# NicholasMilef/UUO-Mocap

Hardware: AMD Instinct MI355X
Metric: mocap frames/sec fitted (300-frame seq, 50 markers) (higher is better)
Workload: dtype f32

## Files before the change

uuo_mocap_amd/_lib.py:

```python
from __future__ import annotations

import ctypes
import os
import re
from ctypes import POINTER, c_char_p, c_float, c_int, c_int32, c_void_p

_HERE = os.path.dirname(os.path.abspath(__file__))
LIB_PATH = os.path.join(_HERE, "libuuo_hip.so")
HEADER_PATH = os.path.join(os.path.dirname(_HERE), "include", "uuo_hip.h")

UUO_STAGE_CHAMFER, UUO_STAGE_MARKER, UUO_STAGE_PART = 0, 1, 2


ABI_VERSION = 3


class UuoProblem(ctypes.Structure):
    _fields_ = [
        ("stage", c_int32), ("F", c_int32), ("M", c_int32),
        ("d_markers", c_void_p), ("d_o_pose", c_void_p), ("d_o_betas", c_void_p), ("d_root", c_void_p),
        ("d_assign", c_void_p), ("d_subset", c_void_p), ("n_subset", c_int32),
        ("w_data", c_float), ("w_pose", c_float), ("w_betas", c_float), ("marker_distance", c_float),
        ("pose_cache_id", ctypes.c_uint64),
        ("w_soft", c_float), ("soft_tau", c_float),
        ("n_corners", c_int32), ("d_bary", c_void_p),
        ("robust_sigma", c_float),
    ]
    w_offsets = None


class _TailFloat:

    size = 4

    def __init__(self, offset: int):
        self.offset = offset

    def __get__(self, obj, owner=None):
        if obj is None:
            return self
        return c_float.from_buffer(obj, self.offset).value

    def __set__(self, obj, value):
        c_float.from_buffer(obj, self.offset).value = value


UuoProblem.w_offsets = _TailFloat(UuoProblem.robust_sigma.offset + 4)
assert UuoProblem.w_offsets.offset + 4 <= ctypes.sizeof(UuoProblem)


class UuoLbfgsOptions(ctypes.Structure):
    _fields_ = [
        ("max_iter", c_int32), ("history_size", c_int32), ("lr", c_float), ("tolerance_grad", c_float),
        ("tolerance_change", c_float), ("max_eval", c_int32), ("verbose", c_int32),
    ]


class UuoLbfgsStats(ctypes.Structure):
    _fields_ = [
        ("n_iter", c_int32), ("n_eval", c_int32), ("first_loss", c_float), ("final_loss", c_float),
        ("stop_reason", c_int32), ("device_ms", c_float),
    ]


class UuoReprojectionProblem(ctypes.Structure):
    _fields_ = [
        ("F", c_int32), ("M", c_int32), ("V", c_int32), ("J", c_int32),
        ("d_markers", c_void_p), ("d_joints0", c_void_p), ("d_verts0", c_void_p), ("d_kp_target", c_void_p),
        ("d_mask", c_void_p), ("focal", c_float * 2), ("center", c_float * 2),
        ("w_reprojection", c_float), ("w_chamfer", c_float),
    ]


EVAL_CALLBACK = ctypes.CFUNCTYPE(None, c_void_p, c_int, c_float, c_void_p)
GATHER_FN = ctypes.CFUNCTYPE(c_int, c_void_p, POINTER(ctypes.c_double), c_int, POINTER(ctypes.c_double))


class UuoShared(ctypes.Structure):
    _fields_ = [("gather", GATHER_FN), ("user", c_void_p), ("rank", c_int32), ("world", c_int32)]


_SIGNATURES = {
    "uuo_last_error": (c_char_p, []),
    "uuo_abi_version": (c_int, []),
    "uuo_model_create": (c_int, [c_void_p] * 7 + [c_int, POINTER(c_void_p)]),
    "uuo_model_destroy": (c_int, [c_void_p]),
    "uuo_model_num_verts": (c_int, [c_void_p]),
    "uuo_model_set_faces": (c_int, [c_void_p, c_void_p, c_int]),
    "uuo_ring_table": (c_int, [c_void_p, c_int, c_int, c_void_p, c_void_p]),
    "uuo_ring_closest_points": (c_int, [c_void_p, c_void_p, c_int, c_int, c_void_p, c_void_p, c_void_p, c_void_p, c_void_p,
                                        c_void_p, c_void_p]),
    "uuo_fit_set_surface": (c_int, [c_void_p, c_int32, c_float]),
    "uuo_fit_surface_corners": (c_int, [c_void_p, c_void_p, c_void_p, c_void_p]),
    "uuo_smpl_forward": (c_int, [c_void_p, c_void_p, c_int, c_void_p, c_void_p, c_int, c_void_p, c_void_p,
                                 c_void_p, c_void_p]),
    "uuo_smpl_backward": (c_int, [c_void_p, c_void_p, c_int, c_void_p, c_void_p, c_int, c_void_p, c_void_p, c_void_p,
                                  c_void_p, c_void_p, c_void_p, c_void_p, c_void_p, c_void_p]),
    "uuo_nn_argmin": (c_int, [c_void_p, c_int, c_int, c_int, c_void_p, c_void_p, c_void_p, c_int, c_void_p,
                              c_void_p, c_void_p]),
    "uuo_rigid_distance_std": (c_int, [c_void_p, c_int, c_int, c_void_p, c_void_p]),
    "uuo_assign_mean_argmin": (c_int, [c_void_p, c_int, c_int, c_int, c_void_p, c_void_p, c_void_p, c_void_p,
                                       c_void_p]),
    "uuo_soft_nn_forward": (c_int, [c_void_p, c_int, c_int, c_int, c_void_p, c_void_p, c_float, c_void_p, c_void_p,
                                    c_void_p, c_void_p]),
    "uuo_soft_nn_backward": (c_int, [c_void_p, c_int, c_int, c_int, c_void_p, c_void_p, c_float, c_void_p, c_void_p,
                                     c_void_p, c_void_p, c_void_p]),
    "uuo_copy_to_host": (c_int, [c_void_p, c_void_p, c_void_p, c_int]),
    "uuo_mesh_closest_points": (c_int, [c_void_p, c_int, c_int, c_int, c_int, c_void_p, c_void_p, c_void_p, c_void_p,
                                        c_void_p, c_void_p, c_void_p]),
    "uuo_fit_create": (c_int, [c_void_p, c_int, c_int, POINTER(c_void_p)]),
    "uuo_fit_destroy": (c_int, [c_void_p]),
    "uuo_assign_segments_argmin": (c_int, [c_void_p, c_int, c_int, c_int, c_int, c_void_p, c_void_p, c_void_p, c_void_p,
                                           c_void_p, c_void_p]),
    "uuo_fit_set_frame_assign": (c_int, [c_void_p, c_void_p]),
    "uuo_fit_set_joint_accel": (c_int, [c_void_p, c_float]),
    "uuo_fit_set_foot_lock": (c_int, [c_void_p, c_float, c_void_p]),
    "uuo_fit_set_floor": (c_int, [c_void_p, c_float, c_float, c_float, c_void_p, c_int, c_int, c_void_p]),
    "uuo_fit_set_capsules": (c_int, [c_void_p, c_float, c_int, c_void_p, c_void_p, c_int, c_void_p]),
    "uuo_fit_set_joint_limits": (c_int, [c_void_p, c_float, c_void_p, c_void_p]),
    "uuo_fit_set_prior_weights": (c_int, [c_void_p, c_void_p]),
    "uuo_problem_num_params": (c_int, [POINTER(UuoProblem)]),
    "uuo_closure_eval": (c_int, [c_void_p, c_void_p, POINTER(UuoProblem), c_void_p, c_void_p, c_void_p, c_void_p]),
    "uuo_lbfgs_solve": (c_int, [c_void_p, c_void_p, POINTER(UuoProblem), c_void_p, POINTER(UuoLbfgsOptions),
                                POINTER(UuoLbfgsStats), c_void_p, c_void_p]),
    "uuo_lbfgs_solve_shared": (c_int, [c_void_p, c_void_p, POINTER(UuoProblem), c_void_p, POINTER(UuoLbfgsOptions),
                                       POINTER(UuoLbfgsStats), POINTER(UuoShared), c_void_p, c_void_p]),
    "uuo_time_closure": (c_int, [c_void_p, c_void_p, POINTER(UuoProblem), c_void_p, c_int, c_int,
                                 POINTER(c_float)]),
    "uuo_lbfgs_minimize": (c_int, [c_void_p, c_int, c_void_p, POINTER(UuoLbfgsOptions), POINTER(UuoLbfgsStats), c_void_p,
                                   c_void_p, c_void_p, c_void_p]),
    "uuo_reprojection_create": (c_int, [POINTER(UuoReprojectionProblem), POINTER(c_void_p)]),
    "uuo_reprojection_destroy": (c_int, [c_void_p]),
    "uuo_reprojection_num_params": (c_int, [POINTER(UuoReprojectionProblem)]),
    "uuo_reprojection_eval": (c_int, [c_void_p, c_void_p, c_void_p, c_void_p, c_void_p, c_void_p, c_void_p]),
    "uuo_reprojection_solve": (c_int, [c_void_p, c_void_p, c_void_p, POINTER(UuoLbfgsOptions), POINTER(UuoLbfgsStats),
                                       c_void_p, c_void_p, c_void_p, c_void_p]),
    "uuo_set_wait_policy": (c_int, [c_int, c_int]),
    "uuo_mailbox_open": (c_int, [c_char_p, c_int32, c_int32, ctypes.c_double, POINTER(c_void_p)]),
    "uuo_mailbox_close": (c_int, [c_void_p]),
    "uuo_mailbox_gather": (c_int, [c_void_p, c_void_p, c_int, c_void_p]),
    "uuo_mailbox_stats": (c_int, [c_void_p, POINTER(ctypes.c_ulonglong), POINTER(ctypes.c_ulonglong)]),
    "uuo_copy_device": (c_int, [c_void_p, c_void_p, c_void_p, ctypes.c_size_t]),
    "uuo_batch_create": (c_int, [c_void_p, c_int, c_int, c_int, c_int, POINTER(c_void_p)]),
    "uuo_batch_destroy": (c_int, [c_void_p]),
    "uuo_batch_solve": (c_int, [c_void_p, c_void_p, POINTER(UuoProblem), POINTER(c_void_p), c_int,
                                POINTER(UuoLbfgsOptions), POINTER(UuoLbfgsStats)]),
    "uuo_batch_part_scores": (c_int, [c_void_p, c_void_p, POINTER(UuoProblem), POINTER(c_void_p), c_int,
                                      POINTER(c_float)]),
}
LIB_DEBUG_PATH = os.path.join(_HERE, "libuuo_hip_debug.so")
_DEBUG_SIGNATURES = {
    "uuo_lbfgs_selftest": (c_int, [c_void_p, c_int, c_int, c_void_p, POINTER(UuoLbfgsOptions),
                                   POINTER(UuoLbfgsStats), c_void_p, c_void_p]),
    "uuo_debug_fit_buffers": (c_int, [c_void_p, c_void_p, c_void_p]),
    "uuo_debug_nn_flags": (c_int, [c_void_p, c_void_p]),
    "uuo_debug_skin16_check": (c_int, [c_void_p, c_int]),
    "uuo_debug_small_coeffs": (c_int, [c_int, c_int, c_int, c_void_p]),
    "uuo_debug_time_small": (c_int, [c_int, c_int, c_int, POINTER(c_float)]),
    "uuo_debug_index_map": (c_int, [c_int, c_int, c_int, c_void_p]),
    "uuo_debug_problem_index_map": (c_int, [POINTER(UuoProblem), c_int, c_void_p]),
    "uuo_debug_bwd_select": (c_int, [c_void_p, c_int, c_void_p, c_void_p]),
    "uuo_debug_last_solve_n": (c_int, [c_void_p]),
    "uuo_debug_staging_script": (c_int, [c_void_p, c_int, ctypes.c_longlong, c_void_p]),
    "uuo_debug_lb_replay_create": (c_int, [c_int, c_int, POINTER(c_void_p)]),
    "uuo_debug_lb_replay_step": (c_int, [c_void_p, c_void_p, c_float, c_float, c_void_p, c_void_p, c_void_p, c_void_p]),
    "uuo_debug_lb_replay_state": (c_int, [c_void_p, c_void_p, c_void_p, c_void_p, c_int, c_void_p, c_void_p]),
    "uuo_debug_lb_replay_destroy": (c_int, [c_void_p]),
}

CLOSURE_FN = ctypes.CFUNCTYPE(c_int, c_void_p, c_void_p, c_void_p, c_void_p, c_void_p)

_lib = None
_lib_debug = None


def header_symbols():
    text = open(HEADER_PATH).read()
    text = re.sub(r"/\*.*?\*/", "", text, flags=re.S)
    names = re.findall(r"\b(uuo_[a-z0-9_]+)\s*\(", text)
    return sorted(set(n for n in names if n != "uuo_eval_callback_t"))


def load():
    global _lib
    if _lib is not None:
        return _lib
    if not os.path.isfile(LIB_PATH):
        raise RuntimeError(
            "libuuo_hip.so is missing (%s): run `python __graft_entry__.py` to build the HIP extension. "
            "There is no CPU fallback for the fitted path." % LIB_PATH)
    lib = ctypes.CDLL(LIB_PATH)
    for name in header_symbols():
        if not hasattr(lib, name):
            raise RuntimeError("libuuo_hip.so does not export %s declared in include/uuo_hip.h" % name)
    for name, (res, args) in _SIGNATURES.items():
        fn = getattr(lib, name)
        fn.restype = res
        fn.argtypes = args
    if lib.uuo_abi_version() != ABI_VERSION:
        raise RuntimeError("libuuo_hip.so has ABI version %d, this package binds version %d: rebuild it "
                           "(python __graft_entry__.py)" % (lib.uuo_abi_version(), ABI_VERSION))
    _lib = lib
    return lib


def load_debug():
    global _lib_debug
    if _lib_debug is not None:
        return _lib_debug
    if not os.path.isfile(LIB_DEBUG_PATH):
        raise RuntimeError("libuuo_hip_debug.so is missing (%s): run `python __graft_entry__.py`" % LIB_DEBUG_PATH)
    lib = ctypes.CDLL(LIB_DEBUG_PATH)
    for name, (res, args) in list(_SIGNATURES.items()) + list(_DEBUG_SIGNATURES.items()):
        fn = getattr(lib, name)
        fn.restype = res
        fn.argtypes = args
    _lib_debug = lib
    return lib


def check(rc: int, what: str = ""):
    if rc != 0:
        msg = load().uuo_last_error()
        raise RuntimeError("%s failed (%d): %s" % (what or "libuuo_hip call", rc, msg.decode() if msg else ""))
```

uuo_mocap_amd/csrc/nn_kernels.hip:

```cpp
#include <cstdlib>

#include "frame_math.h"

#define UUO_INF __builtin_huge_valf()
#include "tri_math.h"

__device__ __forceinline__ float uuo_sqrt_rn(float x) { return __builtin_sqrtf(x); }
__device__ __forceinline__ float uuo_div_rn(float x, float y) { return x / y; }

__device__ __forceinline__ unsigned long long pack_key(float d, unsigned idx) {
  return ((unsigned long long)__float_as_uint(d) << 32) | (unsigned long long)idx;
}

__device__ __forceinline__ float sqdist(float qx, float qy, float qz, float px, float py, float pz) {
  const float dx = __fsub_rn(qx, px), dy = __fsub_rn(qy, py), dz = __fsub_rn(qz, pz);
  return __fadd_rn(__fadd_rn(__fmul_rn(dx, dx), __fmul_rn(dy, dy)), __fmul_rn(dz, dz));
}

__device__ __forceinline__ void nn_body(const float* __restrict__ x, const float* __restrict__ y,
                                        const int* __restrict__ ysub, int P1, int P2, int nc, int S,
                                        unsigned long long* __restrict__ out, int n, int qg, int s) {
  __shared__ float4 sc[64];
  const int lane = threadIdx.x;
  const int q = qg * 64 + lane;
// ... 447 lines not shown
      pf2 T2[6];
      float4 ww;
      unsigned pj;
      float o[3];
      pso_skin(Cf, SB4, sA, sTr, v, cl, o, T2, ww, pj);
      const float rx = o[0] - sTr[0], ry = o[1] - sTr[1];
      if (!valid) o[0] = o[1] = o[2] = 1.0e18f;
      const unsigned cidv = valid ? (unsigned)c : 0xFFFFFFFFu;
      const pf2 ox2 = pf2{o[0], o[0]}, oy2 = pf2{o[1], o[1]}, oz2 = pf2{o[2], o[2]};
      float ax = 0.f, ay = 0.f, az = 0.f;
#pragma unroll
      for (int k = 0; k < QP; ++k) {
        const pf2 dx = qx[k] - ox2, dy = qy[k] - oy2, dz = qz[k] - oz2;
        const pf2 d2 = ((dx * dx) + (dy * dy)) + (dz * dz);
#pragma unroll
        for (int h = 0; h < 2; ++h) {
          const int q = 2 * k + h;
          if (q < QB) {
            const float d = h ? d2.y : d2.x;
            float p = PSO_EXP((uM[q] - d) * kexp) * uW[q];
            p += (cidv == uI[q]) ? c_hard : 0.f;
            ax = fmaf(p, h ? dx.y : dx.x, ax);
            ay = fmaf(p, h ? dy.y : dy.x, ay);
            az = fmaf(p, h ? dz.y : dz.x, az);
          }
        }
      }
      const float g0 = -ax, g1 = -ay, g2 = -az;
      if (!__any((ax != 0.f) | (ay != 0.f) | (az != 0.f))) continue;
      gs[0] += g0;
      gs[1] += g1;
      gs[2] += g2;
      tq += rx * g1 - ry * g0;
      const float dv0 = fmaf(T2[4].x, g2, fmaf(T2[2].x, g1, T2[0].x * g0));
      const float dv1 = fmaf(T2[4].y, g2, fmaf(T2[2].y, g1, T2[0].y * g0));
      const float dv2 = fmaf(T2[5].x, g2, fmaf(T2[3].x, g1, T2[1].x * g0));
      const float* svf = reinterpret_cast<const float*>(sv);
#pragma unroll
      for (int k = 0; k < 10; ++k) db[k] += fmaf(svf[20 + k], dv2, fmaf(svf[10 + k], dv1, svf[k] * dv0));
      const float wv[4] = {ww.x, ww.y, ww.z, ww.w};
#pragma unroll
      for (int n = 0; n < 4; ++n) {
        float* col = sF + ((pj >> (8 * n)) & 0xFFu) * 64u + tid;
        col[0] += wv[n] * g0;
        col[64] += wv[n] * g1;
        col[128] += wv[n] * g2;
      }
    }
  }
  float* pre = a.pre + (size_t)f * UUO_PRE;
  const float r1 = wave_sum_fast(gs[0]), r2 = wave_sum_fast(gs[1]), r3 = wave_sum_fast(gs[2]), r14 = wave_sum_fast(tq);
  float rb[10];
#pragma unroll
  for (int k = 0; k < 10; ++k) rb[k] = wave_sum_fast(db[k]);
  if (tid == 0) {
    pre[0] = loss;
    pre[1] = r1;
    pre[2] = r2;
    pre[3] = r3;
#pragma unroll
    for (int k = 0; k < 10; ++k) pre[4 + k] = rb[k];
    pre[14] = r14;
    pre[15] = 0.f;
  }
  __syncthreads();
  for (int t = tid; t < UUO_NUM_JOINTS * 3; t += 64) {
    float acc = 0.f;
#pragma unroll 8
    for (int i = 0; i < 64; ++i) acc += sF[t * 64 + ((i + t) & 63)];
    pre[16 + t] = acc;
  }
}
template <int QB>
__global__ __launch_bounds__(64) void k_part_soft(PartSoftArgs a) {
  const int f = (int)(blockIdx.x >> 3) * 8 + (int)(blockIdx.x & 7);
  if (f >= a.F) return;
  part_soft_body<QB>(a, f);
}
template <int QB>
__global__ __launch_bounds__(64) void k_part_soft_b(const PartSoftArgs* __restrict__ batch, int count) {
  const int r = (int)(blockIdx.x >> 3);
  const PartSoftArgs a = batch[r % count];
  const int f = (r / count) * 8 + (int)(blockIdx.x & 7);
  if (f >= a.F) return;
  part_soft_body<QB>(a, f);
}

int uuo_launch_part_soft(const uuo_model* m, hipStream_t s, int F, int P1, const float* cache, const float* sb, const float* A,
                         const float* trans, const int32_t* subset, int n_subset, const float* markers,
                         unsigned long long* packed, float* pre, float w_hard, float w_soft, float tau) {
  UUO_REQUIRE(P1 >= 1 && P1 <= NNQ_MAX && subset && n_subset > 0 && F > 0 && pre, "uuo_launch_part_soft: bad arguments");
  UUO_REQUIRE(tau > 0.f && w_soft != 0.f, "uuo_launch_part_soft: needs a positive temperature and a soft weight");
  const double fm = (double)F * (double)P1;
  PartSoftArgs a{{F, P1}, F, m->V, n_subset, P1, subset, cache, sb, A, trans, markers, m->ST, packed, pre,
                 (float)(1.4426950408889634 / (double)tau), (float)((double)tau * 0.6931471805599453), w_hard, w_soft,
                 (float)(2.0 * (double)w_hard / fm), (float)(2.0 * (double)w_soft / fm)};
  if (uuo_record(UUO_OP_PART_SOFT, F, P1, a)) return 0;
  const dim3 grid(8 * ((F + 7) / 8));
  switch (P1) {
#define PSO_CASE(Q) case Q: hipLaunchKernelGGL(k_part_soft<Q>, grid, dim3(64), 0, s, a); break;
    PSO_CASE(1) PSO_CASE(2) PSO_CASE(3) PSO_CASE(4) PSO_CASE(5) PSO_CASE(6) PSO_CASE(7) PSO_CASE(8)
    PSO_CASE(9) PSO_CASE(10) PSO_CASE(11) PSO_CASE(12) PSO_CASE(13) PSO_CASE(14) PSO_CASE(15) PSO_CASE(16)
#undef PSO_CASE
  }
  UUO_HIP_CHECK(hipGetLastError());
  return 0;
}

static int fill_keys(hipStream_t s, unsigned long long* packed, size_t count) {
  FillArgs f{{(int)((count + 255) / 256), 1}, packed, (int)count};
  if (uuo_record(UUO_OP_FILL, f.h.gx, 1, f)) return 0;
  UUO_HIP_CHECK(hipMemsetAsync(packed, 0xFF, count * sizeof(unsigned long long), s));
  return 0;
}

int uuo_launch_nn(hipStream_t s, int N, int P1, int P2, const float* x, const float* y, const int32_t* ysub, int P2s,
                  unsigned long long* packed) {
  const int nc = ysub ? P2s : P2;
  if (nc > 0 && N > 0 && P1 > 0 && P1 <= NNQ_MAX) {
    int S = 1;
    if (N < 1024) S = (1024 + N - 1) / N;
    const int maxS = (nc + 1023) / 1024;
    if (S > maxS) S = maxS;
    if (S < 1 || uuo_recorder) S = 1;
    if (S > 1) {
      const int rc = fill_keys(s, packed, (size_t)N * P1);
      if (rc) return rc;
    }
    NnArgs a{{N, S}, x, y, ysub, P1, P2, nc, S, packed};
    if (uuo_record(UUO_OP_NN_FEWQ, N, S, a)) return 0;
    hipLaunchKernelGGL(k_nn_fewq, dim3(N, S), dim3(256), 0, s, a);
    UUO_HIP_CHECK(hipGetLastError());
    return 0;
  }
  {
    const int rc = fill_keys(s, packed, (size_t)N * P1);
    if (rc) return rc;
  }
  if (nc <= 0 || N <= 0 || P1 <= 0) return 0;
  const int qgroups = (P1 + 63) / 64;
  int S = 1;
  const long waves = (long)N * qgroups;
  if (waves < 4096) S = (int)((4096 + waves - 1) / waves);
  const int maxS = (nc + 255) / 256;
  if (S > maxS) S = maxS;
  if (S < 1) S = 1;
  NnArgs a{{N, qgroups * S}, x, y, ysub, P1, P2, nc, S, packed};
  if (uuo_record(UUO_OP_NN, N, qgroups * S, a)) return 0;
  hipLaunchKernelGGL(k_nn, dim3(N, qgroups, S), dim3(64), 0, s, a);
  UUO_HIP_CHECK(hipGetLastError());
  return 0;
}

#define CULL_CAP 3072
#define CULL_CAP2 1024
#define CULL_MG 64
#define CULL_MAXU 512
#define CULL_UB 4
#define CULL_MAXG 8
#ifndef CULL_SUPER
#define CULL_SUPER 8
#endif
#ifndef CULL_T
#define CULL_T 256
#endif
__device__ __forceinline__ void nn_cull_body(int M, int V, int nunits, int mper, const float* __restrict__ x,
                                             const float* __restrict__ verts, const float* __restrict__ bbox,
                                             unsigned long long* __restrict__ packed, int* __restrict__ stats) {
  __builtin_amdgcn_s_setprio(1);
  __shared__ float sbox[CULL_MAXU * 6];
  __shared__ float smx[CULL_MG * 3];
  __shared__ float sub[CULL_MG];
  __shared__ unsigned long long skey[CULL_MG];
  __shared__ unsigned slist[CULL_CAP];
  __shared__ unsigned scount, scount2;
  const int f = blockIdx.x, tid = threadIdx.x, wave = tid >> 6, lane = tid & 63;
  const int m0 = blockIdx.y * mper;
  const int mg = min(mper, M - m0);
  if (mg <= 0) return;
  const float* vf = verts + (size_t)f * V * 3;
  {
    const float* bf = bbox + (size_t)f * nunits * 6;
    for (int i = tid; i < nunits * 6; i += CULL_T) sbox[i] = bf[i];
  }
  if (tid < mg) {
    const float* px = x + ((size_t)f * M + m0 + tid) * 3;
    const float qx = px[0], qy = px[1], qz = px[2];
    smx[tid * 3] = qx;
    smx[tid * 3 + 1] = qy;
    smx[tid * 3 + 2] = qz;
    unsigned prev = (unsigned)(packed[(size_t)f * M + m0 + tid] & 0xFFFFFFFFull);
    if (prev >= (unsigned)V) prev = 0;
    const float* pv = vf + (size_t)prev * 3;
    const unsigned long long key = pack_key(sqdist(qx, qy, qz, pv[0], pv[1], pv[2]), prev);
    skey[tid] = key;
    sub[tid] = __uint_as_float((unsigned)(key >> 32));
  }
  if (tid == 0) scount = 0u;
  if (tid == 1) scount2 = 0u;
  __syncthreads();
#if CULL_SUPER
  constexpr int NSUP_MAX = (CULL_MAXU + CULL_SUPER - 1) / CULL_SUPER;
  __shared__ float ssup[NSUP_MAX * 6];
  __shared__ unsigned slist2[CULL_CAP2];
  const int nsup = (nunits + CULL_SUPER - 1) / CULL_SUPER;
  for (int sidx = tid; sidx < nsup * 6; sidx += CULL_T) {
    const int sp = sidx / 6, c = sidx - sp * 6;
    const int u0 = sp * CULL_SUPER, u1 = min(nunits, u0 + CULL_SUPER);
    float v = sbox[u0 * 6 + c];
    for (int u = u0 + 1; u < u1; ++u) v = (c < 3) ? fminf(v, sbox[u * 6 + c]) : fmaxf(v, sbox[u * 6 + c]);
    ssup[sidx] = v;
  }
  __syncthreads();
  for (int e = tid; e < nsup * mg; e += CULL_T) {
    const int sp = e / mg, m = e - sp * mg;
    const float* b = ssup + sp * 6;
    const float qx = smx[m * 3], qy = smx[m * 3 + 1], qz = smx[m * 3 + 2];
    const float dx = fmaxf(fmaxf(__fsub_rn(b[0], qx), __fsub_rn(qx, b[3])), 0.f);
    const float dy = fmaxf(fmaxf(__fsub_rn(b[1], qy), __fsub_rn(qy, b[4])), 0.f);
    const float dz = fmaxf(fmaxf(__fsub_rn(b[2], qz), __fsub_rn(qz, b[5])), 0.f);
    const float lb = __fadd_rn(__fadd_rn(__fmul_rn(dx, dx), __fmul_rn(dy, dy)), __fmul_rn(dz, dz));
    if (lb <= sub[m]) {
      const unsigned pos = atomicAdd(&scount2, 1u);
      if (pos < CULL_CAP2) slist2[pos] = ((unsigned)m << 16) | (unsigned)sp;
    }
  }
  __syncthreads();
  const int found2 = (int)scount2;
  if (found2 > CULL_CAP2 && tid == 0) scount = CULL_CAP + 1u;
  for (int e = tid; e < min(found2, CULL_CAP2 + 0) * CULL_SUPER && found2 <= CULL_CAP2; e += CULL_T) {
    const unsigned ent = slist2[e / CULL_SUPER];
    const int m = (int)(ent >> 16), u = (int)(ent & 0xFFFFu) * CULL_SUPER + (e % CULL_SUPER);
    if (u < nunits) {
      const float* b = sbox + u * 6;
      const float qx = smx[m * 3], qy = smx[m * 3 + 1], qz = smx[m * 3 + 2];
      const float dx = fmaxf(fmaxf(__fsub_rn(b[0], qx), __fsub_rn(qx, b[3])), 0.f);
      const float dy = fmaxf(fmaxf(__fsub_rn(b[1], qy), __fsub_rn(qy, b[4])), 0.f);
      const float dz = fmaxf(fmaxf(__fsub_rn(b[2], qz), __fsub_rn(qz, b[5])), 0.f);
      const float lb = __fadd_rn(__fadd_rn(__fmul_rn(dx, dx), __fmul_rn(dy, dy)), __fmul_rn(dz, dz));
      if (lb <= sub[m]) {
        const unsigned pos = atomicAdd(&scount, 1u);
        if (pos < CULL_CAP) slist[pos] = ((unsigned)m << 16) | (unsigned)u;
      }
    }
  }
#else
  for (int u = tid; u < nunits; u += CULL_T) {
    const float* b = sbox + u * 6;
    const float b0 = b[0], b1 = b[1], b2 = b[2], b3 = b[3], b4 = b[4], b5 = b[5];
    unsigned long long mask = 0ull;
#pragma unroll 4
    for (int m = 0; m < mg; ++m) {
      const float qx = smx[m * 3], qy = smx[m * 3 + 1], qz = smx[m * 3 + 2];
      const float dx = fmaxf(fmaxf(__fsub_rn(b0, qx), __fsub_rn(qx, b3)), 0.f);
      const float dy = fmaxf(fmaxf(__fsub_rn(b1, qy), __fsub_rn(qy, b4)), 0.f);
      const float dz = fmaxf(fmaxf(__fsub_rn(b2, qz), __fsub_rn(qz, b5)), 0.f);
      const float lb = __fadd_rn(__fadd_rn(__fmul_rn(dx, dx), __fmul_rn(dy, dy)), __fmul_rn(dz, dz));
      mask |= (lb <= sub[m]) ? (1ull << m) : 0ull;
    }
    const int cnt = __popcll(mask);
    if (cnt) {
      unsigned pos = atomicAdd(&scount, (unsigned)cnt);
      while (mask) {
        const int m = __ffsll((long long)mask) - 1;
        mask &= mask - 1;
        if (pos < CULL_CAP) slist[pos] = ((unsigned)m << 16) | (unsigned)u;
        ++pos;
      }
    }
  }
#endif
  __syncthreads();
  const int found = (int)scount;
  const bool overflow = found > CULL_CAP;
  const int nent = overflow ? nunits * mg : found;
  for (int e0 = wave * 4 * CULL_UB; e0 < nent; e0 += (CULL_T / 64) * 4 * CULL_UB) {
    unsigned long long key[CULL_UB];
    int mm[CULL_UB];
    float vx[CULL_UB], vy[CULL_UB], vz[CULL_UB];
    int vid[CULL_UB];
#pragma unroll
    for (int r = 0; r < CULL_UB; ++r) {
      const int e = e0 + 4 * r + (lane >> 4);
      mm[r] = 0;
      vid[r] = -1;
      vx[r] = vy[r] = vz[r] = 0.f;
      if (e < nent) {
        int u;
        if (overflow) {
          u = e / mg;
          mm[r] = e - u * mg;
        } else {
          const unsigned ent = slist[e];
          mm[r] = (int)(ent >> 16);
          u = (int)(ent & 0xFFFFu);
        }
        const int vtx = u * 16 + (lane & 15);
        if (vtx < V) {
          const float* pv = vf + (size_t)vtx * 3;
          vx[r] = pv[0];
          vy[r] = pv[1];
          vz[r] = pv[2];
          vid[r] = vtx;
        }
      }
    }
#pragma unroll
    for (int r = 0; r < CULL_UB; ++r) {
      const int m = mm[r];
      key[r] = (vid[r] >= 0)
                   ? pack_key(sqdist(smx[m * 3], smx[m * 3 + 1], smx[m * 3 + 2], vx[r], vy[r], vz[r]), (unsigned)vid[r])
                   : ~0ull;
#pragma unroll
      for (int off = 8; off >= 1; off >>= 1) {
        const unsigned long long o = __shfl_xor(key[r], off, 16);
        key[r] = o < key[r] ? o : key[r];
      }
      if ((lane & 15) == 0 && key[r] != ~0ull) atomicMin(&skey[m], key[r]);
    }
  }
  __syncthreads();
  if (tid < mg) packed[(size_t)f * M + m0 + tid] = skey[tid];
  if (tid == 0 && stats) stats[f * CULL_MAXG + blockIdx.y] = overflow ? -found : found;
}

struct NnCullArgs {
  UuoGridHdr h;
  int M, V, nunits, mper;
  uuo_gptr<const float> x;
  uuo_gptr<const float> verts;
  uuo_gptr<const float> bbox;
  uuo_gptr<unsigned long long> packed;
  uuo_gptr<int> stats;
};
__global__ __launch_bounds__(CULL_T) void k_nn_cull(NnCullArgs a) {
  nn_cull_body(a.M, a.V, a.nunits, a.mper, a.x, a.verts, a.bbox, a.packed, a.stats);
}
__global__ __launch_bounds__(CULL_T) void k_nn_cull_b(const NnCullArgs* __restrict__ batch) {
  UUO_BATCH_PICK(NnCullArgs, batch)
  nn_cull_body(a.M, a.V, a.nunits, a.mper, a.x, a.verts, a.bbox, a.packed, a.stats);
}

int uuo_launch_nn_cull(hipStream_t s, int F, int M, int V, int nunits, const float* markers, const float* verts,
                       const float* bbox, unsigned long long* packed, int* stats) {
  if (F <= 0 || M <= 0) return 0;
  UUO_REQUIRE(nunits <= CULL_MAXU, "uuo_launch_nn_cull: too many vertex units for the LDS box table");
  int G = (M + CULL_MG - 1) / CULL_MG;
  while (G < CULL_MAXG && (long)F * G < 1024 && (M + G) / (G + 1) >= 8) ++G;
  const int mper = (M + G - 1) / G;
  UUO_REQUIRE(mper <= CULL_MG && G <= CULL_MAXG, "uuo_launch_nn_cull: too many markers per frame for the pruned search");
  NnCullArgs a{{F, G}, M, V, nunits, mper, markers, verts, bbox, packed, stats};
  if (uuo_record(UUO_OP_NN_CULL, F, G, a)) return 0;
  hipLaunchKernelGGL(k_nn_cull, dim3(F, G), dim3(CULL_T), 0, s, a);
  UUO_HIP_CHECK(hipGetLastError());
  return 0;
}

int uuo_batched_launch_nn(int op, hipStream_t s, const void* d_args, int count, int gx, int gy) {
  if (op == UUO_OP_FILL) {
    hipLaunchKernelGGL(k_fill_keys_b, dim3(gx, gy, count), dim3(256), 0, s, (const FillArgs*)d_args);
  } else if (op == UUO_OP_NN) {
    hipLaunchKernelGGL(k_nn_b, dim3(gx, gy, count), dim3(64), 0, s, (const NnArgs*)d_args);
  } else if (op == UUO_OP_NN_FEWQ) {
    hipLaunchKernelGGL(k_nn_fewq_b, dim3(gx, gy, count), dim3(256), 0, s, (const NnArgs*)d_args);
  } else if (op == UUO_OP_NN_CULL) {
    hipLaunchKernelGGL(k_nn_cull_b, dim3(gx, gy, count), dim3(CULL_T), 0, s, (const NnCullArgs*)d_args);
  } else if (op == UUO_OP_PART_FWD) {
    const dim3 grid(8 * ((gx + 7) / 8) * count);
    const PartFwdArgs* pa = (const PartFwdArgs*)d_args;
    switch (gy) {
#define PFW_CASE(Q) case Q: hipLaunchKernelGGL(k_part_fwd_b<Q>, grid, dim3(PFW_T), 0, s, pa, count); break;
      PFW_CASE(1) PFW_CASE(2) PFW_CASE(3) PFW_CASE(4) PFW_CASE(5) PFW_CASE(6) PFW_CASE(7) PFW_CASE(8)
      PFW_CASE(9) PFW_CASE(10) PFW_CASE(11) PFW_CASE(12) PFW_CASE(13) PFW_CASE(14) PFW_CASE(15) PFW_CASE(16)
#undef PFW_CASE
      default: UUO_REQUIRE(false, "batched k_part_fwd: markers per frame out of range");
    }
  } else if (op == UUO_OP_PART_SOFT) {
    const dim3 grid(8 * ((gx + 7) / 8) * count);
    const PartSoftArgs* pa = (const PartSoftArgs*)d_args;
    switch (gy) {
#define PSO_CASE(Q) case Q: hipLaunchKernelGGL(k_part_soft_b<Q>, grid, dim3(64), 0, s, pa, count); break;
      PSO_CASE(1) PSO_CASE(2) PSO_CASE(3) PSO_CASE(4) PSO_CASE(5) PSO_CASE(6) PSO_CASE(7) PSO_CASE(8)
      PSO_CASE(9) PSO_CASE(10) PSO_CASE(11) PSO_CASE(12) PSO_CASE(13) PSO_CASE(14) PSO_CASE(15) PSO_CASE(16)
#undef PSO_CASE
      default: UUO_REQUIRE(false, "batched k_part_soft: markers per frame out of range");
    }
  } else {
    return 1;
  }
  UUO_HIP_CHECK(hipGetLastError());
  return 0;
}

__global__ void k_nn_unpack(int count, const unsigned long long* __restrict__ packed, float* __restrict__ dist,
                            int32_t* __restrict__ idx) {
  const int i = blockIdx.x * blockDim.x + threadIdx.x;
  if (i >= count) return;
  const unsigned long long k = packed[i];
  if (dist) dist[i] = __uint_as_float((unsigned)(k >> 32));
  if (idx) idx[i] = (int32_t)(unsigned)(k & 0xFFFFFFFFull);
}

int uuo_launch_nn_unpack(hipStream_t s, int count, const unsigned long long* packed, float* dist, int32_t* idx) {
  if (count <= 0) return 0;
  hipLaunchKernelGGL(k_nn_unpack, dim3((count + 255) / 256), dim3(256), 0, s, count, packed, dist, idx);
  UUO_HIP_CHECK(hipGetLastError());
  return 0;
}

extern "C" int uuo_nn_argmin(void* stream, int N, int P1, int P2, const float* d_x, const float* d_y,
                             const int32_t* d_y_subset, int P2s, float* d_dist, int32_t* d_idx, void* d_ws) {
  UUO_REQUIRE(d_x && d_y && d_ws, "uuo_nn_argmin: null argument (workspace of N*P1 uint64 is required)");
  UUO_REQUIRE(N >= 0 && P1 >= 0 && P2 >= 0, "uuo_nn_argmin: negative size");
  hipStream_t s = (hipStream_t)stream;
  int rc = uuo_launch_nn(s, N, P1, P2, d_x, d_y, d_y_subset, P2s, (unsigned long long*)d_ws);
  if (rc) return rc;
  return uuo_launch_nn_unpack(s, N * P1, (const unsigned long long*)d_ws, d_dist, d_idx);
}

#define ASSIGN_MG 4
#define ASSIGN_FC 32
#define ASSIGN_U 4
__global__ __launch_bounds__(256) void k_assign(int F, int M, int V, const float* __restrict__ verts,
                                                 const float* __restrict__ markers,
                                                 const unsigned char* __restrict__ valid, int count,
                                                 unsigned long long* __restrict__ out) {
  __shared__ float sm[ASSIGN_FC][ASSIGN_MG * 3];
  __shared__ unsigned char sv[ASSIGN_FC];
  const int v = blockIdx.x * 256 + threadIdx.x;
  const int vc = v < V ? v : V - 1;
  const int m0 = blockIdx.y * ASSIGN_MG;
  float acc[ASSIGN_MG];
#pragma unroll
  for (int g = 0; g < ASSIGN_MG; ++g) acc[g] = 0.f;
  for (int f0 = 0; f0 < F; f0 += ASSIGN_FC) {
    const int nf = min(ASSIGN_FC, F - f0);
    __syncthreads();
    for (int i = threadIdx.x; i < nf * ASSIGN_MG * 3; i += 256) {
      const int ff = i / (ASSIGN_MG * 3), r = i - ff * (ASSIGN_MG * 3), g = r / 3, c = r - g * 3;
      sm[ff][r] = (m0 + g < M) ? markers[((size_t)(f0 + ff) * M + m0 + g) * 3 + c] : 0.f;
    }
    if (threadIdx.x < nf) sv[threadIdx.x] = valid[f0 + threadIdx.x];
    __syncthreads();
    for (int q0 = 0; q0 < nf; q0 += ASSIGN_U) {
      float px[ASSIGN_U], py[ASSIGN_U], pz[ASSIGN_U];
#pragma unroll
      for (int u = 0; u < ASSIGN_U; ++u) {
        const int ff = min(q0 + u, nf - 1);
        const float* pv = verts + ((size_t)(f0 + ff) * V + vc) * 3;
        px[u] = pv[0]; py[u] = pv[1]; pz[u] = pv[2];
      }
#pragma unroll
      for (int u = 0; u < ASSIGN_U; ++u) {
        const int ff = q0 + u;
        if (ff < nf && sv[ff]) {
#pragma unroll
          for (int g = 0; g < ASSIGN_MG; ++g) {
            const float d2 = sqdist(px[u], py[u], pz[u], sm[ff][g * 3], sm[ff][g * 3 + 1], sm[ff][g * 3 + 2]);
            acc[g] = __fadd_rn(acc[g], uuo_sqrt_rn(d2));
          }
        }
      }
    }
  }
#pragma unroll
  for (int g = 0; g < ASSIGN_MG; ++g) {
    if (m0 + g < M) {
      unsigned long long key = ~0ull;
      if (v < V) key = pack_key(uuo_div_rn(acc[g], (float)count), (unsigned)v);
#pragma unroll
      for (int off = 32; off >= 1; off >>= 1) {
        const unsigned long long o = __shfl_xor(key, off, 64);
        key = o < key ? o : key;
      }
      if ((threadIdx.x & 63) == 0 && key != ~0ull) atomicMin(&out[m0 + g], key);
    }
  }
}

int uuo_launch_assign(hipStream_t s, int F, int M, int V, const float* verts, const float* markers,
                      const uint8_t* valid, int32_t* idx, unsigned long long* packed) {
  unsigned char* h = (unsigned char*)malloc(F);
  if (!h) return -12;
  hipError_t e = hipMemcpyAsync(h, valid, F, hipMemcpyDeviceToHost, s);
  if (e == hipSuccess) e = hipStreamSynchronize(s);
  if (e != hipSuccess) {
    free(h);
    uuo_set_error(std::string("uuo_assign_mean_argmin: ") + hipGetErrorString(e));
    return -5;
  }
  int count = 0;
  for (int f = 0; f < F; ++f) count += h[f] ? 1 : 0;
  free(h);
  UUO_REQUIRE(count > 0, "uuo_assign_mean_argmin: no valid frame");
  UUO_HIP_CHECK(hipMemsetAsync(packed, 0xFF, (size_t)M * sizeof(unsigned long long), s));
  hipLaunchKernelGGL(k_assign, dim3((V + 255) / 256, (M + ASSIGN_MG - 1) / ASSIGN_MG), dim3(256), 0, s, F, M, V, verts,
                     markers, valid, count, packed);
  UUO_HIP_CHECK(hipGetLastError());
  return uuo_launch_nn_unpack(s, M, packed, nullptr, idx);
}

extern "C" int uuo_assign_mean_argmin(void* stream, int F, int M, int V, const float* d_verts, const float* d_markers,
                                      const uint8_t* d_valid, int32_t* d_idx, void* d_ws) {
  UUO_REQUIRE(d_verts && d_markers && d_valid && d_idx && d_ws, "uuo_assign_mean_argmin: null argument");
  UUO_REQUIRE(F > 0 && M > 0 && V > 0, "uuo_assign_mean_argmin: sizes must be positive");
  return uuo_launch_assign((hipStream_t)stream, F, M, V, d_verts, d_markers, d_valid, d_idx, (unsigned long long*)d_ws);
}

__device__ __forceinline__ void assign_seg_flush(float acc, int n, int sid, int v, int V, unsigned long long* __restrict__ out) {
  unsigned long long key = ~0ull;
  if (v < V) key = pack_key(uuo_div_rn(acc, (float)n), (unsigned)v);
#pragma unroll
  for (int off = 32; off >= 1; off >>= 1) {
    const unsigned long long o = __shfl_xor(key, off, 64);
    key = o < key ? o : key;
  }
  if ((threadIdx.x & 63) == 0 && key != ~0ull) atomicMin(&out[sid], key);
}

// ... 657 lines not shown
```

Baseline: 1448.

## Shrink nn-cull LDS footprint with dynamic sizing and batched unit tests

Replaces the large static LDS tables in the culled nearest-neighbour kernel (full box table, 3072-entry list) with dynamically sized shared memory. Super-box bounds are now built with DPP lane reductions from registers instead of an LDS box copy. Fine unit boxes are re-read from global memory and tested in batches of 1024, so no overflow fallback is needed, and a dense case switches to full enumeration. The goal is to raise occupancy and drop the redundant LDS staging, at the cost of extra global box reads and more barrier-separated batch passes.

After: 1504 (median of 6 runs). +3.9%, better.

```diff
diff --git a/uuo_mocap_amd/_lib.py b/uuo_mocap_amd/_lib.py
--- a/uuo_mocap_amd/_lib.py
+++ b/uuo_mocap_amd/_lib.py
@@ -154,6 +154,8 @@
                                    POINTER(UuoLbfgsStats), c_void_p, c_void_p]),
     "uuo_debug_fit_buffers": (c_int, [c_void_p, c_void_p, c_void_p]),
     "uuo_debug_nn_flags": (c_int, [c_void_p, c_void_p]),
+    "uuo_debug_nn_cull_geometry": (c_int, [c_int, c_int, c_int, c_void_p]),
+    "uuo_debug_nn_cull": (c_int, [c_void_p, c_int, c_int, c_int] + [c_void_p] * 5),
     "uuo_debug_skin16_check": (c_int, [c_void_p, c_int]),
     "uuo_debug_small_coeffs": (c_int, [c_int, c_int, c_int, c_void_p]),
     "uuo_debug_time_small": (c_int, [c_int, c_int, c_int, POINTER(c_float)]),
diff --git a/uuo_mocap_amd/csrc/nn_kernels.hip b/uuo_mocap_amd/csrc/nn_kernels.hip
--- a/uuo_mocap_amd/csrc/nn_kernels.hip
+++ b/uuo_mocap_amd/csrc/nn_kernels.hip
@@ -623,36 +623,56 @@
   return 0;
 }
 
-#define CULL_CAP 3072
-#define CULL_CAP2 1024
+#define CULL_CAP 1024
 #define CULL_MG 64
 #define CULL_MAXU 512
 #define CULL_UB 4
 #define CULL_MAXG 8
-#ifndef CULL_SUPER
 #define CULL_SUPER 8
-#endif
 #ifndef CULL_T
 #define CULL_T 256
 #endif
+#define CULL_AB (CULL_CAP / CULL_T)
+static_assert(CULL_CAP % CULL_T == 0, "a batch of unit tests is a whole number of block passes");
+static_assert((CULL_MAXU + CULL_SUPER - 1) / CULL_SUPER <= 64 && CULL_MG <= 64, "a (marker, super-box) pair packs into 12 bits");
+__host__ __device__ constexpr int cull_lds_bytes(int mper, int nsup) {
+  return 8 * mper + 24 * nsup + 12 * mper + 4 * mper + 4 * CULL_CAP + 2 * ((mper * nsup + 1) & ~1);
+}
+extern __shared__ __align__(8) unsigned char cull_lds[];
+__device__ __forceinline__ float cull_box_lb(float b0, float b1, float b2, float b3, float b4, float b5, float qx, float qy,
+                                             float qz) {
+  const float dx = fmaxf(fmaxf(__fsub_rn(b0, qx), __fsub_rn(qx, b3)), 0.f);
+  const float dy = fmaxf(fmaxf(__fsub_rn(b1, qy), __fsub_rn(qy, b4)), 0.f);
+  const float dz = fmaxf(fmaxf(__fsub_rn(b2, qz), __fsub_rn(qz, b5)), 0.f);
+  return __fadd_rn(__fadd_rn(__fmul_rn(dx, dx), __fmul_rn(dy, dy)), __fmul_rn(dz, dz));
+}
 __device__ __forceinline__ void nn_cull_body(int M, int V, int nunits, int mper, const float* __restrict__ x,
                                              const float* __restrict__ verts, const float* __restrict__ bbox,
                                              unsigned long long* __restrict__ packed, int* __restrict__ stats) {
   __builtin_amdgcn_s_setprio(1);
-  __shared__ float sbox[CULL_MAXU * 6];
-  __shared__ float smx[CULL_MG * 3];
-  __shared__ float sub[CULL_MG];
-  __shared__ unsigned long long skey[CULL_MG];
-  __shared__ unsigned slist[CULL_CAP];
-  __shared__ unsigned scount, scount2;
+  const int nsup = (nunits + CULL_SUPER - 1) / CULL_SUPER;
+  unsigned long long* skey = (unsigned long long*)cull_lds;
+  float* ssup = (float*)(skey + mper);
+  float* smx = ssup + nsup * 6;
+  float* sub = smx + mper * 3;
+  unsigned* slist = (unsigned*)(sub + mper);
+  unsigned short* slist2 = (unsigned short*)(slist + CULL_CAP);
+  __shared__ unsigned scount[2], scount2;
   const int f = blockIdx.x, tid = threadIdx.x, wave = tid >> 6, lane = tid & 63;
   const int m0 = blockIdx.y * mper;
   const int mg = min(mper, M - m0);
   if (mg <= 0) return;
   const float* vf = verts + (size_t)f * V * 3;
-  {
-    const float* bf = bbox + (size_t)f * nunits * 6;
-    for (int i = tid; i < nunits * 6; i += CULL_T) sbox[i] = bf[i];
+  const float* bf = bbox + (size_t)f * nunits * 6;
+  static_assert(CULL_MAXU <= 2 * CULL_T && CULL_SUPER == 8, "two passes of one unit per thread, a super-box = 8 lanes");
+  float w[2][6];
+#pragma unroll
+  for (int p = 0; p < 2; ++p) {
+    if (p * CULL_T < nunits) {
+      const float2* pb = (const float2*)(bf + min(p * CULL_T + tid, nunits - 1) * 6);
+      const float2 lo = pb[0], mid = pb[1], hi = pb[2];
+      w[p][0] = lo.x, w[p][1] = lo.y, w[p][2] = mid.x, w[p][3] = mid.y, w[p][4] = hi.x, w[p][5] = hi.y;
+    }
   }
   if (tid < mg) {
     const float* px = x + ((size_t)f * M + m0 + tid) * 3;
@@ -667,132 +687,118 @@
     skey[tid] = key;
     sub[tid] = __uint_as_float((unsigned)(key >> 32));
   }
-  if (tid == 0) scount = 0u;
-  if (tid == 1) scount2 = 0u;
-  __syncthreads();
-#if CULL_SUPER
-  constexpr int NSUP_MAX = (CULL_MAXU + CULL_SUPER - 1) / CULL_SUPER;
-  __shared__ float ssup[NSUP_MAX * 6];
-  __shared__ unsigned slist2[CULL_CAP2];
-  const int nsup = (nunits + CULL_SUPER - 1) / CULL_SUPER;
-  for (int sidx = tid; sidx < nsup * 6; sidx += CULL_T) {
-    const int sp = sidx / 6, c = sidx - sp * 6;
-    const int u0 = sp * CULL_SUPER, u1 = min(nunits, u0 + CULL_SUPER);
-    float v = sbox[u0 * 6 + c];
-    for (int u = u0 + 1; u < u1; ++u) v = (c < 3) ? fminf(v, sbox[u * 6 + c]) : fmaxf(v, sbox[u * 6 + c]);
-    ssup[sidx] = v;
+  if (tid == 0) scount[0] = scount[1] = scount2 = 0u;
+  {
+#pragma unroll
+    for (int p = 0; p < 2; ++p) {
+      if (p * CULL_T < nunits) {
+#pragma unroll
+        for (int c = 0; c < 6; ++c) {
+          float v = w[p][c];
+          v = (c < 3) ? fminf(v, dpp_rot<0xB1>(v)) : fmaxf(v, dpp_rot<0xB1>(v));
+          v = (c < 3) ? fminf(v, dpp_rot<0x4E>(v)) : fmaxf(v, dpp_rot<0x4E>(v));
+          w[p][c] = (c < 3) ? fminf(v, dpp_rot<0x141>(v)) : fmaxf(v, dpp_rot<0x141>(v));
+        }
+        const int sp = (p * CULL_T + tid) / CULL_SUPER;
+        if ((tid & (CULL_SUPER - 1)) == 0 && sp < nsup) {
+#pragma unroll
+          for (int c = 0; c < 6; ++c) ssup[sp * 6 + c] = w[p][c];
+        }
+      }
+    }
   }
   __syncthreads();
   for (int e = tid; e < nsup * mg; e += CULL_T) {
     const int sp = e / mg, m = e - sp * mg;
     const float* b = ssup + sp * 6;
-    const float qx = smx[m * 3], qy = smx[m * 3 + 1], qz = smx[m * 3 + 2];
-    const float dx = fmaxf(fmaxf(__fsub_rn(b[0], qx), __fsub_rn(qx, b[3])), 0.f);
-    const float dy = fmaxf(fmaxf(__fsub_rn(b[1], qy), __fsub_rn(qy, b[4])), 0.f);
-    const float dz = fmaxf(fmaxf(__fsub_rn(b[2], qz), __fsub_rn(qz, b[5])), 0.f);
-    const float lb = __fadd_rn(__fadd_rn(__fmul_rn(dx, dx), __fmul_rn(dy, dy)), __fmul_rn(dz, dz));
-    if (lb <= sub[m]) {
-      const unsigned pos = atomicAdd(&scount2, 1u);
-      if (pos < CULL_CAP2) slist2[pos] = ((unsigned)m << 16) | (unsigned)sp;
-    }
+    const float lb = cull_box_lb(b[0], b[1], b[2], b[3], b[4], b[5], smx[m * 3], smx[m * 3 + 1], smx[m * 3 + 2]);
+    if (lb <= sub[m]) slist2[atomicAdd(&scount2, 1u)] = (unsigned short)((m << 6) | sp);
   }
   __syncthreads();
   const int found2 = (int)scount2;
-  if (found2 > CULL_CAP2 && tid == 0) scount = CULL_CAP + 1u;
-  for (int e = tid; e < min(found2, CULL_CAP2 + 0) * CULL_SUPER && found2 <= CULL_CAP2; e += CULL_T) {
-    const unsigned ent = slist2[e / CULL_SUPER];
-    const int m = (int)(ent >> 16), u = (int)(ent & 0xFFFFu) * CULL_SUPER + (e % CULL_SUPER);
-    if (u < nunits) {
-      const float* b = sbox + u * 6;
-      const float qx = smx[m * 3], qy = smx[m * 3 + 1], qz = smx[m * 3 + 2];
-      const float dx = fmaxf(fmaxf(__fsub_rn(b[0], qx), __fsub_rn(qx, b[3])), 0.f);
-      const float dy = fmaxf(fmaxf(__fsub_rn(b[1], qy), __fsub_rn(qy, b[4])), 0.f);
-      const float dz = fmaxf(fmaxf(__fsub_rn(b[2], qz), __fsub_rn(qz, b[5])), 0.f);
-      const float lb = __fadd_rn(__fadd_rn(__fmul_rn(dx, dx), __fmul_rn(dy, dy)), __fmul_rn(dz, dz));
-      if (lb <= sub[m]) {
-        const unsigned pos = atomicAdd(&scount, 1u);
-        if (pos < CULL_CAP) slist[pos] = ((unsigned)m << 16) | (unsigned)u;
-      }
-    }
-  }
-#else
-  for (int u = tid; u < nunits; u += CULL_T) {
-    const float* b = sbox + u * 6;
-    const float b0 = b[0], b1 = b[1], b2 = b[2], b3 = b[3], b4 = b[4], b5 = b[5];
-    unsigned long long mask = 0ull;
-#pragma unroll 4
-    for (int m = 0; m < mg; ++m) {
-      const float qx = smx[m * 3], qy = smx[m * 3 + 1], qz = smx[m * 3 + 2];
-      const float dx = fmaxf(fmaxf(__fsub_rn(b0, qx), __fsub_rn(qx, b3)), 0.f);
-      const float dy = fmaxf(fmaxf(__fsub_rn(b1, qy), __fsub_rn(qy, b4)), 0.f);
-      const float dz = fmaxf(fmaxf(__fsub_rn(b2, qz), __fsub_rn(qz, b5)), 0.f);
-      const float lb = __fadd_rn(__fadd_rn(__fmul_rn(dx, dx), __fmul_rn(dy, dy)), __fmul_rn(dz, dz));
-      mask |= (lb <= sub[m]) ? (1ull << m) : 0ull;
-    }
-    const int cnt = __popcll(mask);
-    if (cnt) {
-      unsigned pos = atomicAdd(&scount, (unsigned)cnt);
-      while (mask) {
-        const int m = __ffsll((long long)mask) - 1;
-        mask &= mask - 1;
-        if (pos < CULL_CAP) slist[pos] = ((unsigned)m << 16) | (unsigned)u;
-        ++pos;
-      }
-    }
-  }
-#endif
-  __syncthreads();
-  const int found = (int)scount;
-  const bool overflow = found > CULL_CAP;
-  const int nent = overflow ? nunits * mg : found;
-  for (int e0 = wave * 4 * CULL_UB; e0 < nent; e0 += (CULL_T / 64) * 4 * CULL_UB) {
-    unsigned long long key[CULL_UB];
-    int mm[CULL_UB];
-    float vx[CULL_UB], vy[CULL_UB], vz[CULL_UB];
-    int vid[CULL_UB];
-#pragma unroll
-    for (int r = 0; r < CULL_UB; ++r) {
-      const int e = e0 + 4 * r + (lane >> 4);
-      mm[r] = 0;
-      vid[r] = -1;
-      vx[r] = vy[r] = vz[r] = 0.f;
-      if (e < nent) {
+  const bool enumerate = 4 * found2 > 3 * nsup * mg;
+  const int ntest = enumerate ? 0 : found2 * CULL_SUPER;
+  int found = 0;
+  for (int base = 0, batch = 0;; base += CULL_CAP, ++batch) {
+    int nent = nunits * mg;
+    if (!enumerate) {
+      float bx[CULL_AB][6];
+      int tm[CULL_AB], tu[CULL_AB];
+#pragma unroll
+      for (int r = 0; r < CULL_AB; ++r) {
+        const int e = base + r * CULL_T + tid;
+        tu[r] = -1;
+        tm[r] = 0;
+#pragma unroll
+        for (int c = 0; c < 6; ++c) bx[r][c] = 0.f;
+        if (e < ntest) {
+          const unsigned ent = slist2[e / CULL_SUPER];
+          const int u = (int)(ent & 63u) * CULL_SUPER + (e % CULL_SUPER);
+          if (u < nunits) {
+            const float2* pb = (const float2*)(bf + u * 6);
+            const float2 lo = pb[0], mid = pb[1], hi = pb[2];
+            bx[r][0] = lo.x, bx[r][1] = lo.y, bx[r][2] = mid.x, bx[r][3] = mid.y, bx[r][4] = hi.x, bx[r][5] = hi.y;
+            tm[r] = (int)(ent >> 6);
+            tu[r] = u;
+          }
+        }
+      }
+      unsigned* cnt = &scount[batch & 1];
+#pragma unroll
+      for (int r = 0; r < CULL_AB; ++r) {
+        const int m = tm[r];
+        const float lb = cull_box_lb(bx[r][0], bx[r][1], bx[r][2], bx[r][3], bx[r][4], bx[r][5], smx[m * 3], smx[m * 3 + 1],
+                                     smx[m * 3 + 2]);
+        if (tu[r] >= 0 && lb <= sub[m]) slist[atomicAdd(cnt, 1u)] = ((unsigned)m << 16) | (unsigned)tu[r];
+      }
+      __syncthreads();
+      nent = (int)*cnt;
+      found += nent;
+      if (tid == 0) scount[(batch + 1) & 1] = 0u;
+    }
+    for (int e0 = wave * 4 * CULL_UB; e0 < nent; e0 += (CULL_T / 64) * 4 * CULL_UB) {
+      unsigned long long key[CULL_UB];
+      int mm[CULL_UB];
+      float vx[CULL_UB], vy[CULL_UB], vz[CULL_UB];
+      int vid[CULL_UB];
+#pragma unroll
+      for (int r = 0; r < CULL_UB; ++r) {
+        const int e = e0 + 4 * r + (lane >> 4), ec = min(e, nent - 1);
         int u;
-        if (overflow) {
-          u = e / mg;
-          mm[r] = e - u * mg;
+        if (enumerate) {
+          u = ec / mg;
+          mm[r] = ec - u * mg;
         } else {
-          const unsigned ent = slist[e];
+          const unsigned ent = slist[ec];
           mm[r] = (int)(ent >> 16);
           u = (int)(ent & 0xFFFFu);
         }
         const int vtx = u * 16 + (lane & 15);
-        if (vtx < V) {
-          const float* pv = vf + (size_t)vtx * 3;
-          vx[r] = pv[0];
-          vy[r] = pv[1];
-          vz[r] = pv[2];
-          vid[r] = vtx;
+        const float* pv = vf + (size_t)min(vtx, V - 1) * 3;
+        vx[r] = pv[0];
+        vy[r] = pv[1];
+        vz[r] = pv[2];
+        vid[r] = (e < nent && vtx < V) ? vtx : -1;
+      }
+#pragma unroll
+      for (int r = 0; r < CULL_UB; ++r) {
+        const int m = mm[r];
+        key[r] = (vid[r] >= 0)
+                     ? pack_key(sqdist(smx[m * 3], smx[m * 3 + 1], smx[m * 3 + 2], vx[r], vy[r], vz[r]), (unsigned)vid[r])
+                     : ~0ull;
+#pragma unroll
+        for (int off = 8; off >= 1; off >>= 1) {
+          const unsigned long long o = __shfl_xor(key[r], off, 16);
+          key[r] = o < key[r] ? o : key[r];
         }
-      }
-    }
-#pragma unroll
-    for (int r = 0; r < CULL_UB; ++r) {
-      const int m = mm[r];
-      key[r] = (vid[r] >= 0)
-                   ? pack_key(sqdist(smx[m * 3], smx[m * 3 + 1], smx[m * 3 + 2], vx[r], vy[r], vz[r]), (unsigned)vid[r])
-                   : ~0ull;
-#pragma unroll
-      for (int off = 8; off >= 1; off >>= 1) {
-        const unsigned long long o = __shfl_xor(key[r], off, 16);
-        key[r] = o < key[r] ? o : key[r];
-      }
-      if ((lane & 15) == 0 && key[r] != ~0ull) atomicMin(&skey[m], key[r]);
-    }
-  }
-  __syncthreads();
+        if ((lane & 15) == 0 && key[r] != ~0ull) atomicMin(&skey[m], key[r]);
+      }
+    }
+    __syncthreads();
+    if (base + CULL_CAP >= ntest) break;
+  }
   if (tid < mg) packed[(size_t)f * M + m0 + tid] = skey[tid];
-  if (tid == 0 && stats) stats[f * CULL_MAXG + blockIdx.y] = overflow ? -found : found;
+  if (tid == 0 && stats) stats[f * CULL_MAXG + blockIdx.y] = enumerate ? -(nunits * mg) : found;
 }
 
 struct NnCullArgs {
@@ -812,20 +818,41 @@
   nn_cull_body(a.M, a.V, a.nunits, a.mper, a.x, a.verts, a.bbox, a.packed, a.stats);
 }
 
+static void cull_geometry(int F, int M, int nunits, int* G_out, int* mper_out, int* lds_out) {
+  int G = (M + CULL_MG - 1) / CULL_MG;
+  while (G < CULL_MAXG && (long)F * G < 1024 && (M + G) / (G + 1) >= 8) ++G;
+  *G_out = G;
+  *mper_out = (M + G - 1) / G;
+  *lds_out = cull_lds_bytes(*mper_out, (nunits + CULL_SUPER - 1) / CULL_SUPER);
+}
+
 int uuo_launch_nn_cull(hipStream_t s, int F, int M, int V, int nunits, const float* markers, const float* verts,
                        const float* bbox, unsigned long long* packed, int* stats) {
   if (F <= 0 || M <= 0) return 0;
-  UUO_REQUIRE(nunits <= CULL_MAXU, "uuo_launch_nn_cull: too many vertex units for the LDS box table");
-  int G = (M + CULL_MG - 1) / CULL_MG;
-  while (G < CULL_MAXG && (long)F * G < 1024 && (M + G) / (G + 1) >= 8) ++G;
-  const int mper = (M + G - 1) / G;
+  UUO_REQUIRE(nunits >= 1 && nunits <= CULL_MAXU, "uuo_launch_nn_cull: too many vertex units for the box table");
+  int G, mper, lds;
+  cull_geometry(F, M, nunits, &G, &mper, &lds);
   UUO_REQUIRE(mper <= CULL_MG && G <= CULL_MAXG, "uuo_launch_nn_cull: too many markers per frame for the pruned search");
   NnCullArgs a{{F, G}, M, V, nunits, mper, markers, verts, bbox, packed, stats};
   if (uuo_record(UUO_OP_NN_CULL, F, G, a)) return 0;
-  hipLaunchKernelGGL(k_nn_cull, dim3(F, G), dim3(CULL_T), 0, s, a);
+  hipLaunchKernelGGL(k_nn_cull, dim3(F, G), dim3(CULL_T), lds, s, a);
   UUO_HIP_CHECK(hipGetLastError());
   return 0;
 }
+
+#ifdef UUO_DEBUG_HOOKS
+extern "C" int uuo_debug_nn_cull_geometry(int F, int M, int nunits, int* out) {
+  UUO_REQUIRE(F > 0 && M > 0 && nunits >= 1 && nunits <= CULL_MAXU && out, "uuo_debug_nn_cull_geometry: bad arguments");
+  cull_geometry(F, M, nunits, &out[0], &out[1], &out[2]);
+  out[3] = CULL_CAP;
+  return 0;
+}
+extern "C" int uuo_debug_nn_cull(void* stream, int F, int M, int V, const float* d_markers, const float* d_verts,
+                                 const float* d_bbox, unsigned long long* d_keys, int* d_stats) {
+  UUO_REQUIRE(V > 0 && d_markers && d_verts && d_bbox && d_keys, "uuo_debug_nn_cull: bad arguments");
+  return uuo_launch_nn_cull((hipStream_t)stream, F, M, V, (V + 15) / 16, d_markers, d_verts, d_bbox, d_keys, d_stats);
+}
+#endif
 
 int uuo_batched_launch_nn(int op, hipStream_t s, const void* d_args, int count, int gx, int gy) {
   if (op == UUO_OP_FILL) {
@@ -835,7 +862,8 @@
   } else if (op == UUO_OP_NN_FEWQ) {
     hipLaunchKernelGGL(k_nn_fewq_b, dim3(gx, gy, count), dim3(256), 0, s, (const NnArgs*)d_args);
   } else if (op == UUO_OP_NN_CULL) {
-    hipLaunchKernelGGL(k_nn_cull_b, dim3(gx, gy, count), dim3(CULL_T), 0, s, (const NnCullArgs*)d_args);
+    hipLaunchKernelGGL(k_nn_cull_b, dim3(gx, gy, count), dim3(CULL_T), cull_lds_bytes(CULL_MG, CULL_MAXU / CULL_SUPER), s,
+                       (const NnCullArgs*)d_args);
   } else if (op == UUO_OP_PART_FWD) {
     const dim3 grid(8 * ((gx + 7) / 8) * count);
     const PartFwdArgs* pa = (const PartFwdArgs*)d_args;
```
